# EPFL-VILAB/omnidata

Hardware: AMD Instinct MI355X
Metric: images/sec (384x384) DPT-Hybrid surface-normal inference (higher is better)
Workload: dtype bf16; 1 GPU; DPT-Hybrid-384 normal, batch 32/GPU, bf16, 1xMI355X (BASELINE.json configs[1]); batch_per_gpu=32, global_batch=32, parallelism=replicas x1 (no collective in the loop), ranks_seen=1, inflight=1

## Files before the change

include/dptx.h:

```cpp
#ifndef DPTX_H_
#define DPTX_H_

#include <stddef.h>
#include <stdint.h>

#ifdef __cplusplus
extern "C" {
#endif

typedef struct dptx_engine* dptx_handle;

enum {
  DPTX_OK = 0,
  DPTX_E_INVALID = -1,
  DPTX_E_KEY = -2,
  DPTX_E_HIP = -3,
  DPTX_E_NODEVICE = -4,
  DPTX_E_ALLOC = -5
};

enum { DPTX_DTYPE_BF16 = 0, DPTX_DTYPE_FP16 = 1, DPTX_DTYPE_BF16X3 = 2,
       DPTX_DTYPE_FP16X3 = 3, DPTX_DTYPE_MIXED = 4,
       DPTX_DTYPE_FP8 = 5 };
enum { DPTX_GROUP_RESNET = 1,
// ... 221 lines not shown
int dptx_op_cls_rows(int32_t dtype, const float* cls, const float* pos, float* X, int32_t B, int32_t S, int32_t C, void* X16,
                     float* row_stats, void* X8, float q_scale, void* stream);
int dptx_debug_set_trace(void* dev_buf);
int dptx_debug_arena_fill(dptx_handle h, int32_t byte_value);
int dptx_debug_arena_read(dptx_handle h, void* dst_host, size_t offset, size_t bytes);
int dptx_debug_arena_layout(dptx_handle h, char* dst, size_t capacity);
int dptx_debug_arena_checksums(dptx_handle h, void* out_dev, int32_t capacity, void* stream);
int dptx_debug_set_gemm_flags(int32_t flags);
int dptx_op_conv_fp8(const void* X8, const void* Wt8, const float* bias, const void* R, void* Y, void* Y8, int32_t B,
                     int32_t H, int32_t W, int32_t Cin, int32_t Cout, int32_t ksize, int32_t stride, int32_t pad_t,
                     int32_t pad_l, int32_t Ho, int32_t Wo, int32_t act, int32_t q_relu, float out_scale, void* stream);
int dptx_op_conv_groupnorm(int32_t dtype, const void* X, const void* Wt, void* Yraw, const float* gamma, const float* beta,
                           const void* R, void* Y, int32_t B, int32_t H, int32_t W, int32_t Cin, int32_t Cout,
                           int32_t ksize, int32_t stride, int32_t pad_t, int32_t pad_l, int32_t Ho, int32_t Wo,
                           int32_t relu, float eps, void* scratch_f32, void* stream);
int dptx_op_upsample2x(int32_t dtype, const void* X, void* Y, int32_t B, int32_t H, int32_t W,
                       int32_t C, void* stream);
int dptx_op_gemm_ln(int32_t dtype, const void* A, const void* W, const float* bias, void* C, int32_t M, int32_t N, int32_t K,
                    int32_t act, const float* ln_stats, const float* ln_colsum, int32_t ln_nblk, float ln_eps, void* stream);
int dptx_op_gemm_stream(int32_t dtype, const void* A, const void* W, const float* bias, void* C, float* row_stats, int32_t M,
                        int32_t N, int32_t K, void* stream);
int dptx_op_gemm_stream32(int32_t dtype, const void* A, const void* W, const float* bias, float* X, void* C16, float* row_stats,
                          int32_t M, int32_t N, int32_t K, void* stream);
int dptx_op_head_tail(int32_t dtype, const void* H0, const void* W2, const float* b2, const float* w4,
                      const float* b4, float* y, int32_t B, int32_t Hs, int32_t Ws, int32_t C,
                      int32_t relu_out, void* stream);

typedef struct dptx_unet_engine* dptx_unet_handle;
typedef struct dptx_unet_config {
  int32_t out_channels;
// ... 40 lines not shown
```

omnidata_amd/csrc/conv1x1.hip:

```cpp
#include "gemm_impl.h"

namespace dptx {

constexpr int C1_STG_PITCH = 144;
constexpr int C1_STG_WAVE = 16 * C1_STG_PITCH;
constexpr int C1_WAVES = 4;

template <int KT, int BN>
constexpr size_t conv1x1_smem_bytes() {
  return (size_t)KT * BN * 128 + (size_t)C1_WAVES * KT * 32 * 128 + (size_t)C1_WAVES * C1_STG_WAVE;
}

template <int DT, int KT, int BN>
__global__ __launch_bounds__(64 * C1_WAVES, KT <= 2 ? 2 : 1) void conv1x1_stream_kernel(const GemmParams p) {
#if defined(__HIP_DEVICE_COMPILE__)
  constexpr int NSUB = BN / 64;
  constexpr int KS = KT * 4;
  constexpr int W_BYTES = KT * BN * 128;
  constexpr int A_WAVE = KT * 32 * 128;
  extern __shared__ __attribute__((aligned(16))) char smem[];

  const int tid = threadIdx.x;
  const int lane = tid & 63;
  const int wave = __builtin_amdgcn_readfirstlane(tid >> 6);
  const int lr = lane & 31, lh = lane >> 5;

  const int npan = p.N / BN;
  const int x = (int)blockIdx.x & 7, l = (int)blockIdx.x >> 3;
// ... 35 lines not shown
    }
  };

  if (rb < rb_total) issue_a(rb);
  for (int idx = wave; idx < KT * (BN / 8); idx += C1_WAVES) {
    const int kt = idx / (BN / 8), rg = idx - kt * (BN / 8);
    const int row = rg * 8 + r0;
    const unsigned vo = (unsigned)(((long long)(n0 + row) * p.ldw + kt * 64 + (kc ^ ((row >> 1) & 7)) * 8) * 2);
    __builtin_amdgcn_raw_ptr_buffer_load_lds(rsrcW, (__attribute__((address_space(3))) void*)(sw + kt * (BN * 128) + rg * 1024), 16, vo,
                                             0, 0, 0);
  }
  float bias_c[NSUB][2];
#pragma unroll
  for (int s = 0; s < NSUB; ++s)
#pragma unroll
    for (int j = 0; j < 2; ++j) bias_c[s][j] = p.bias != nullptr ? p.bias[n0 + s * 64 + j * 32 + lr] : 0.f;
  asm volatile("s_waitcnt vmcnt(0)" ::: "memory");
  __syncthreads();

  const int swz = (lr >> 1) & 7;
  const unsigned sel = (lr & 1) ? 0x03020706u : 0x05040100u;
  const int cn = lane & 7, rr = lane >> 3;

  for (; rb < rb_total; rb += slots) {
    const int m0 = rb * 32;
    u32x4_t af[KS];
#pragma unroll
    for (int ks = 0; ks < KS; ++ks)
      af[ks] = *(const u32x4_t*)(sa + (ks >> 2) * 4096 + lr * 128 + (((2 * (ks & 3) + lh) ^ swz) << 4));
    asm volatile("s_waitcnt lgkmcnt(0)" ::: "memory");
    const bool prefetch = rb + slots < rb_total;
    if (prefetch) issue_a(rb + slots);

#pragma unroll
    for (int s = 0; s < NSUB; ++s) {
      f32x16_t acc[1][2];
#pragma unroll
      for (int j = 0; j < 2; ++j)
#pragma unroll
        for (int r = 0; r < 16; ++r) acc[0][j][r] = 0.f;
// ... 3 lines not shown
#pragma unroll
        for (int q = 0; q < 4; ++q)
#pragma unroll
          for (int j = 0; j < 2; ++j)
            bf[q][j] = *(const u32x4_t*)(sw + kt * (BN * 128) + (s * 64 + j * 32 + lr) * 128 + (((2 * q + lh) ^ swz) << 4));
        __builtin_amdgcn_sched_barrier(0);
#pragma unroll
        for (int q = 0; q < 4; ++q)
#pragma unroll
          for (int j = 0; j < 2; ++j) acc[0][j] = T16<DT>::mfma32(af[kt * 4 + q], bf[q][j], acc[0][j]);
      }
      if (s == 0) {
        __builtin_amdgcn_sched_barrier(0);
        asm volatile("s_waitcnt vmcnt(0)" ::: "memory");
      }
      if (p.gn_part != nullptr) gn_records<1, 2>(p, m0, n0 + s * 64, 0, 0, lr, lh, acc);

#pragma unroll
      for (int h = 0; h < 2; ++h) {
        asm volatile("" ::: "memory");
        __builtin_amdgcn_wave_barrier();
#pragma unroll
        for (int j = 0; j < 2; ++j)
#pragma unroll
          for (int t = 0; t < 4; ++t) {
            float v0 = acc[0][j][8 * h + 2 * t] + bias_c[s][j], v1 = acc[0][j][8 * h + 2 * t + 1] + bias_c[s][j];
            if (p.act == 1) { v0 = fmaxf(v0, 0.f); v1 = fmaxf(v1, 0.f); }
            const uint32_t own = T16<DT>::pack2(v0, v1);
            const uint32_t nb = (uint32_t)__builtin_amdgcn_update_dpp(0, (int)own, 0xB1, 0xf, 0xf, false);
            const uint32_t o = __builtin_amdgcn_perm(nb, own, sel);
            const int rl = ((2 * t) & 3) + (lr & 1) + 8 * (t >> 1) + 4 * lh;
            *(uint32_t*)(stg + rl * C1_STG_PITCH + (j * 32 + (lr & ~1)) * 2) = o;
          }
        asm volatile("" ::: "memory");
        __builtin_amdgcn_wave_barrier();
#pragma unroll
        for (int pp = 0; pp < 2; ++pp) {
          const int rl = rr + 8 * pp;
          const u32x4_t d = *(const u32x4_t*)(stg + rl * C1_STG_PITCH + cn * 16);
          const int m = m0 + 16 * h + rl;
          if (m < p.M) *(u32x4_t*)((uint16_t*)p.C + (long long)(p.c_row_off + m) * p.ldc + (n0 + s * 64 + cn * 8)) = d;
        }
      }
    }
  }
#endif
}

bool conv1x1_stream_eligible(int mode, const GemmParams& p) {
  if (mode != MODE_BF16 && mode != MODE_FP16) return false;
  if (p.ksz != 1 || p.pad_t != 0 || p.pad_l != 0 || (p.stride != 1 && p.stride != 2)) return false;
  if (p.K != p.Cin || (p.K != 64 && p.K != 128 && p.K != 256) || p.N % 64 != 0) return false;
  if (p.a_fp32 || p.c_fp32 || p.epi2 || p.a_relu || p.R1 != nullptr || p.R2 != nullptr || p.bias_per_img) return false;
  if (p.c_rpi != 0x7fffffff || p.C8 != nullptr || p.C16 != nullptr || p.out_scale != 0.f) return false;
  if (p.row_stats != nullptr || p.ln_stats != nullptr || (p.act != 0 && p.act != 1)) return false;
  if (p.ldc % 8 != 0 || p.a_pix_stride % 8 != 0 || p.a_off % 8 != 0 || p.a_img_stride % 8 != 0) return false;
  if (p.a_bytes <= 0 || p.a_bytes >= (1ll << 31) || (long long)p.N * p.ldw * 2 >= (1ll << 31) || p.M >= (1 << 23)) return false;
  return true;
}

bool conv1x1_stream_adopted(const GemmParams& p) {
  if (p.stride != 1) return false;
  if (p.K == 64) return p.N == 256 || p.N == 64;
  if (p.K == 128) return p.N == 512;
  if (p.K == 256) return p.N == 64 || p.N == 128 || (p.N == 256 && p.a_rpi >= 48 * 48);
  return false;
}

template <int DT, int KT, int BN>
static hipError_t launch_c1(const GemmParams& p, hipStream_t stream) {
  constexpr size_t smem = conv1x1_smem_bytes<KT, BN>();
  static_assert(smem <= 160 * 1024 && (KT > 2 || 2 * smem <= 160 * 1024), "two blocks per CU at K <= 128");
  const int npan = p.N / BN;
  const int rb_total = (p.M + 31) / 32;
  const int want = (rb_total + C1_WAVES - 1) / C1_WAVES;
  int cap = (KT <= 2 ? 512 : 256) / npan;
  if (cap < 8) cap = 8;
  int groups = want < cap ? want : cap;
  groups = (groups + 7) / 8 * 8;
  auto k = conv1x1_stream_kernel<DT, KT, BN>;
  set_smem_attr(k, smem);
  hipLaunchKernelGGL(k, dim3(groups * npan), dim3(64 * C1_WAVES), smem, stream, p);
  return hipGetLastError();
}

template <int DT>
static hipError_t launch_c1_dt(const GemmParams& p, hipStream_t stream) {
  if (p.K == 64) {
    if (p.N % 256 == 0) return launch_c1<DT, 1, 256>(p, stream);
    if (p.N % 128 == 0) return launch_c1<DT, 1, 128>(p, stream);
    return launch_c1<DT, 1, 64>(p, stream);
  }
  if (p.K == 128) return p.N % 128 == 0 ? launch_c1<DT, 2, 128>(p, stream) : launch_c1<DT, 2, 64>(p, stream);
  return p.N % 128 == 0 ? launch_c1<DT, 4, 128>(p, stream) : launch_c1<DT, 4, 64>(p, stream);
}

hipError_t launch_conv1x1_stream(int mode, const GemmParams& p, hipStream_t stream) {
  if (!conv1x1_stream_eligible(mode, p)) return hipErrorInvalidValue;
  return mode == MODE_BF16 ? launch_c1_dt<DT_BF16>(p, stream) : launch_c1_dt<DT_FP16>(p, stream);
}

}
```

omnidata_amd/csrc/engine.hip:

```cpp
#include <hip/hip_runtime.h>

#include <algorithm>
#include <cmath>
#include <cstdio>
#include <chrono>
#include <cstring>
#include <map>
#include <memory>
#include <string>
#include <unordered_map>
#include <vector>

#include "../../include/dptx.h"
#include "kernels.h"

using namespace dptx;

namespace {

constexpr int IMG = 384;
constexpr int S_TOK = 577;
constexpr int FEAT = 256;
const int STAGE_DEPTH[3] = {3, 4, 9};
const int STAGE_OUT[3] = {256, 512, 1024};
// ... 353 lines not shown
  double cat_ms[4] = {0, 0, 0, 0};
  int64_t cat_launches[4] = {0, 0, 0, 0};
  double cat_macs[4] = {0, 0, 0, 0};

  static constexpr int MAX_STREAMS = 4;
  int n_streams = 2;
  bool auto_streams = false, split_tuned = false, split_on = false;
  float tune_ms_single = 0.f, tune_ms_split = 0.f;
  int force_schedule = -1;
  int half_batch = 0;
  size_t half_region = 0;
  hipStream_t sub_stream[MAX_STREAMS] = {nullptr, nullptr, nullptr, nullptr};
  hipEvent_t ev_fork = nullptr, ev_join[MAX_STREAMS] = {nullptr, nullptr, nullptr, nullptr};
  int max_h = 384, max_w = 384;
  Buf pos_alt;
  Buf sraw, stem, S[3], T1, T2, PA, PB, DS, part[4], X, Hn, QKV, AO, F1, R3, R4, L3, T4, L4, clsb, lrn[4], tA, tB,
      tC, P[4], H0, H0U, H1, lnst;
  std::vector<std::pair<std::string, const Buf*>> arena_bufs;

  int fail(int code, const std::string& m) {
    err = m;
    return code;
  }
  const void* w(const std::string& key) const { return d_blob + packed_off.at(key); }
  const float* f(const std::string& key) const { return (const float*)(d_blob + packed_off.at(key)); }
  BlobHeader blob_header() const {
    BlobHeader hd;
    memset(&hd, 0, sizeof hd);
    memcpy(hd.magic, "DPTXBLOB", 8);
    hd.version = BLOB_VERSION;
    hd.dtype = cfg.dtype; hd.backbone = backbone; hd.dual_task = cfg.dual_task; hd.num_channels = cfg.num_channels;
// ... 35 lines not shown
    if (half) b.off2 = off; else { b.off = off; b.bytes = bytes; e->arena_bufs.push_back({name, &b}); }
    off += bytes;
  };
  auto idx = [](const char* name, int i) { return name + std::to_string(i); };
  take("sraw", e->sraw, B * p2 * 64, 2);
  take("stem", e->stem, B * p4 * 64, 2);
  take("S0", e->S[0], B * p4 * 256, 2);
  take("S1", e->S[1], B * p8 * 512, 2);
  take("S2", e->S[2], B * p16 * 1024, 2);
  take("T1", e->T1, B * p4 * 128, 2);
  take("T2", e->T2, B * p4 * 64, 2);
  take("PA", e->PA, B * p4 * 256, 2);
  take("PB", e->PB, B * p4 * 256, 2);
  take("DS", e->DS, B * p4 * 256, 2);
  for (int i = 0; i < 4; ++i) take(idx("part", i), e->part[i], B * (std::max(p2 / 256, p4 / 32) + 64) * 64, 4);
  take("X", e->X, B * S * DV, 4);
  take("lnst", e->lnst, B * S * 8 * 2, 4);
  take("Hn", e->Hn, B * S * DV, 2);
  take("QKV", e->QKV, B * S * 3 * DV, 2);
  take("AO", e->AO, B * S * DV, 2);
  take("F1", e->F1, B * S * (size_t)e->dm, 2);
  take("R3", e->R3, B * p16 * DV, 2);
  take("R4", e->R4, B * p16 * DV, 2);
  take("L3", e->L3, B * p16 * DV, 2);
  take("T4", e->T4, B * p16 * DV, 2);
  take("L4", e->L4, B * p32 * DV, 2);
  take("clsb", e->clsb, B * DV, 4);
  take("pos_alt", e->pos_alt, S * DV, 4);
  const size_t rn_px[4] = {p4, p8, p16, p32};
  for (int i = 0; i < 4; ++i) take(idx("lrn", i), e->lrn[i], B * rn_px[i] * FEAT, 2);
// ... 308 lines not shown
  }

  static bool gn_fusable(int HW) { return HW % 32 == 0; }
  void gn_stats(const void* X, float* part, int HW, int C) { chk(launch_gn_stats(dt, X, part, B, HW, C, e->pl, st), "gn_stats", 2); }
  void gn_apply(void* X, const std::string& nkey, float* part, int HW, int C, int relu, const void* R = nullptr,
                const std::string& rkey = "", const float* rpart = nullptr) {
    GnParams g{};
    g.nrec = gn_fusable(HW) ? HW / 32 : 0;
    g.X = X; g.Y = X; g.gamma = e->f(nkey + ".weight"); g.beta = e->f(nkey + ".bias"); g.partial = part;
    g.R = R;
    if (!rkey.empty()) { g.r_gamma = e->f(rkey + ".weight"); g.r_beta = e->f(rkey + ".bias"); g.r_partial = rpart; }
    g.B = B; g.HW = HW; g.C = C; g.relu = relu; g.eps = 1e-5f;
    chk(launch_gn_apply(dt, g, e->pl, st), nkey.c_str(), 2);
  }

  void rcu(const std::string& p, const void* x, int H, int W, void* tmp, void* out, const GemmOpt& o) {
    const int mid_lo = e->mixed() ? (int)e->layer_reads_lo(p + "conv2.weight", cur_group) : -1;
    conv(x, H, W, FEAT, p + "conv1.weight", 3, 1, 1, 1, H, W, FEAT, tmp,
         GemmOpt().bias(e->f(p + "conv1.bias")).act(1).a_relu(1).q(e->fp8_use(p + "conv2.weight") ? 1 : 0).out_lo(mid_lo));
    conv(tmp, H, W, FEAT, p + "conv2.weight", 3, 1, 1, 1, H, W, FEAT, out,
         GemmOpt().bias(e->f(p + "conv2.bias")).R1(x).R2(o.R2_).q(o.q_).out_lo(e->mixed() ? o.out_lo_ : -1));
  }

  int forward(const void* x, void* y, void* y2);
};

int Run::forward(const void* x, void* y, void* y2) {
  dptx_engine* E = e;
  E->taps.clear();
  E->event_cat.clear();
// ... 43 lines not shown
      const int stride = (b == 0) ? STAGE_STRIDE[s] : 1;
      const int Ho = H / stride, Wo = Wd / stride;
      void* out = (b == STAGE_DEPTH[s] - 1) ? (void*)A(E->S[s]) : (void*)((b & 1) ? A(E->PB) : A(E->PA));
      const bool f_in = gn_fusable(H * Wd), f_out = gn_fusable(Ho * Wo);
      if (b == 0) {
        conv(cur, H, Wd, cin, p + "downsample.conv.weight", 1, stride, 0, 0, Ho, Wo, cout, A(E->DS), GemmOpt().gn_part(f_out ? part3 : nullptr));
        if (!f_out) gn_stats(A(E->DS), part3, Ho * Wo, cout);
      }
      conv(cur, H, Wd, cin, p + "conv1.weight", 1, 1, 0, 0, H, Wd, mid, A(E->T1), GemmOpt().gn_part(f_in ? part0 : nullptr));
      if (!f_in) gn_stats(A(E->T1), part0, H * Wd, mid);
      gn_apply(A(E->T1), p + "norm1", part0, H * Wd, mid, 1);
      const int pad = (stride == 1) ? 1 : 0;
      conv(A(E->T1), H, Wd, mid, p + "conv2.weight", 3, stride, pad, pad, Ho, Wo, mid, A(E->T2), GemmOpt().gn_part(f_out ? part1 : nullptr));
      if (!f_out) gn_stats(A(E->T2), part1, Ho * Wo, mid);
      gn_apply(A(E->T2), p + "norm2", part1, Ho * Wo, mid, 1);
      conv(A(E->T2), Ho, Wo, mid, p + "conv3.weight", 1, 1, 0, 0, Ho, Wo, cout, out, GemmOpt().gn_part(f_out ? part2 : nullptr));
      if (!f_out) gn_stats(out, part2, Ho * Wo, cout);
      if (b == 0)
        gn_apply(out, p + "norm3", part2, Ho * Wo, cout, 1, A(E->DS), p + "downsample.norm", part3);
      else
        gn_apply(out, p + "norm3", part2, Ho * Wo, cout, 1, cur);
      cur = out;
      H = Ho;
      Wd = Wo;
      cin = cout;
    }
    const char* names[3] = {"s0", "s1", "s2"};
    tap(names[s], cur, H, Wd, cout);
  }
  }

  float* X = (float*)A(E->X);
  float* lnst = (float*)A(E->lnst);
  const int ln_nblk = D_VIT / 128;
  const bool s16 = E->stream16;
  group(DPTX_GROUP_EMBED);
// ... 913 lines not shown
```

omnidata_amd/csrc/gemm.hip:

```cpp
#include "gemm_impl.h"

namespace dptx {

hipError_t launch_gemm_16(int dt, const GemmParams& p, hipStream_t stream) {
  return dt == DT_BF16 ? launch_dt<DT_BF16, 1>(p, stream) : launch_gemm_fp16(p, stream);
}

void gemm_params_dense(GemmParams& p, int M, int N, int K) {
  p = GemmParams{};
  p.M = M; p.N = N; p.K = K; p.ldw = K;
  p.a_rpi = M > 0 ? M : 1; p.Wout = p.a_rpi; p.Hin = 1; p.Win = p.a_rpi; p.Cin = K; p.a_pix_stride = K;
  p.a_img_stride = 0; p.a_off = 0; p.ksz = 1; p.stride = 1; p.pad_t = 0; p.pad_l = 0;
  p.c_rpi = 0x7fffffff; p.c_img_rows = 0; p.c_row_off = 0; p.ldc = N;
  p.a_bytes = (long long)M * K * 2;
}

void gemm_params_conv(GemmParams& p, int B, int Hin, int Win, int Cin, int Cout, int ksz, int stride, int pad_t, int pad_l,
                      int Hout, int Wout, int a_elem_bytes) {
  p = GemmParams{};
  p.M = B * Hout * Wout; p.N = Cout; p.K = ksz * ksz * Cin; p.ldw = p.K;
  p.a_rpi = Hout * Wout; p.Wout = Wout; p.Hin = Hin; p.Win = Win; p.Cin = Cin; p.a_pix_stride = Cin;
  p.a_img_stride = (long long)Hin * Win * Cin; p.a_off = 0; p.ksz = ksz; p.stride = stride; p.pad_t = pad_t; p.pad_l = pad_l;
  p.c_rpi = 0x7fffffff; p.c_img_rows = 0; p.c_row_off = 0; p.ldc = Cout;
  p.a_bytes = (long long)B * Hin * Win * Cin * a_elem_bytes;
  p.k_tap_fast = (ksz == 3 && Cin >= 512) ? 1 : 0;
}

static thread_local long long* g_trace = nullptr;
void gemm_set_trace(long long* dev_buf) { g_trace = dev_buf; }
static thread_local int g_debug_flags = 0;
void gemm_set_debug_flags(int flags) { g_debug_flags = flags; }
static thread_local float g_cu_share = 1.0f;
void gemm_set_cu_share(float share) { g_cu_share = share > 0.f && share <= 1.f ? share : 1.0f; }

hipError_t launch_gemm(int mode, const GemmParams& p0, hipStream_t stream) {
  GemmParams p = p0;
  p.trace = g_trace;
  p.debug_flags = g_debug_flags;
  if (p.cu_share <= 0.f) p.cu_share = g_cu_share;
  p.a_rpi_rcp = 1.0f / (float)(p.a_rpi > 0 ? p.a_rpi : 1);
  p.wout_rcp = 1.0f / (float)(p.Wout > 0 ? p.Wout : 1);
  if (p.gn_part != nullptr && (p.gn_hw % 32 != 0 || p.N % 32 != 0 || p.gn_cpg != p.N / 32 || p.gn_cpg < 2 || p.gn_cpg > 32 ||
                               (p.gn_cpg & (p.gn_cpg - 1)) != 0 || p.bias != nullptr || p.act != 0))
    return hipErrorInvalidValue;
  if (p.row_stats != nullptr && (p.N % 128 != 0 || p.stats_nblk != 8 || p.N / 128 > 8)) return hipErrorInvalidValue;
  if (p.ln_stats != nullptr && (p.R1 != nullptr || p.R2 != nullptr || p.bias_per_img || p.ln_colsum == nullptr || (p.ln_nblk != 6 && p.ln_nblk != 8) ||
// ... 19 lines not shown
```

omnidata_amd/csrc/kernels.h:

```cpp
#pragma once
#include <hip/hip_runtime.h>
#include <stdint.h>

#include "common.h"

namespace dptx {

void ensure_dyn_smem(const void* kernel, size_t bytes);

struct GemmParams {
  const void* A;
  const void* W;
  void* C;
  const float* bias;
  const void* R1;
  const void* R2;
  int M, N, K;
  int ldw;
  int a_rpi, Wout, Hin, Win, Cin, a_pix_stride;
  long long a_img_stride, a_off;
  long long a_bytes;
  int ksz, stride, pad_t, pad_l;
  int c_rpi, c_img_rows, c_row_off, ldc;
  int r2_bcast;
// ... 13 lines not shown
  int gn_hw, gn_blocks, gn_cpg;
  void* C8;
  int q_relu;
  float out_scale, q_scale;
  const float* out_scale_v;
  void* C16;
  float* row_stats;
  int stats_nblk;
  const float* ln_stats;
  const float* ln_colsum;
  int ln_nblk;
  float ln_eps, ln_inv_dim;
  long long* trace;
  int debug_flags;
  float a_rpi_rcp, wout_rcp;
};

void gemm_params_dense(GemmParams& p, int M, int N, int K);
void gemm_params_conv(GemmParams& p, int B, int Hin, int Win, int Cin, int Cout, int ksz, int stride, int pad_t, int pad_l,
                      int Hout, int Wout, int a_elem_bytes);
hipError_t launch_gemm(int dtype, const GemmParams& p, hipStream_t stream);
void gemm_set_trace(long long* dev_buf);
void gemm_set_debug_flags(int flags);
bool conv1x1_stream_eligible(int mode, const GemmParams& p);
bool conv1x1_stream_adopted(const GemmParams& p);
hipError_t launch_conv1x1_stream(int mode, const GemmParams& p, hipStream_t stream);
void gemm_set_cu_share(float share);

hipError_t launch_attention(int mode, const void* qkv, void* out, int B, int S, int heads, Planes pl, hipStream_t stream);

hipError_t launch_layernorm(int mode, const float* x, const float* gamma, const float* beta, void* y,
                            int M, int C, float eps, Planes pl, hipStream_t stream);

struct GnParams {
  const void* X; void* Y;
  const float* gamma; const float* beta;
  float* partial;
  const void* R;
  const float* r_gamma; const float* r_beta; const float* r_partial;
  int B, HW, C, relu;
  float eps;
  int nrec;
};
int gn_chunks(int HW, int C);
hipError_t launch_gn_stats(int mode, const void* X, float* partial, int B, int HW, int C, Planes pl, hipStream_t stream);
hipError_t launch_gn_apply(int mode, const GnParams& p, Planes pl, hipStream_t stream);
hipError_t launch_gn_relu_maxpool(int mode, const void* X, void* Y, const float* gamma, const float* beta,
                                  const float* partial, int B, int H, int W, int C, float eps, Planes pl, hipStream_t stream);

hipError_t launch_stem_conv(int mode, const void* x, int io, const void* Wt, void* y, int B, int H, int W, Planes pl,
                            hipStream_t stream);

hipError_t launch_upsample2x(int mode, const void* X, void* Y, int B, int H, int W, int C, Planes pl, hipStream_t stream,
                             void* Y8 = nullptr, float q_scale = 1.0f, bool out_hi_only = false);
hipError_t launch_amax(int mode, const void* X, size_t n, int relu, unsigned* amax_bits, hipStream_t stream);

hipError_t launch_nonfinite_scan(int mode, const void* X, size_t n, unsigned* flag, hipStream_t stream);

// ... 23 lines not shown
```

omnidata_amd/csrc/norm.hip:

```cpp
#include "common.h"
#include "kernels.h"

namespace dptx {

template <int DT, int PL, int VPL>
__global__ __launch_bounds__(256) void layernorm_kernel(const float* __restrict__ x, const float* __restrict__ gamma,
                                                        const float* __restrict__ beta, uint16_t* __restrict__ y,
                                                        int M, int C, float eps, long long plane) {
  const int lane = threadIdx.x & 63;
  const int row = blockIdx.x * 4 + (threadIdx.x >> 6);
  if (row >= M) return;
  const float* xr = x + (long long)row * C;
  float4 v[VPL];
  float s = 0.f;
#pragma unroll
  for (int j = 0; j < VPL; ++j) {
    v[j] = *(const float4*)(xr + (j * 64 + lane) * 4);
    s += (v[j].x + v[j].y) + (v[j].z + v[j].w);
  }
  const float mean = wave_sum(s) / (float)C;
  float q = 0.f;
#pragma unroll
  for (int j = 0; j < VPL; ++j) {
    const float a = v[j].x - mean, b = v[j].y - mean, c = v[j].z - mean, d = v[j].w - mean;
// ... 123 lines not shown
  __syncthreads();
  if (tid < GN_G) {
    double ss = 0.0, qq = 0.0;
#pragma unroll
    for (int sl = 0; sl < 8; ++sl) { ss += sred[sl][tid][0]; qq += sred[sl][tid][1]; }
    const double n = (double)HW * (double)cpg;
    const double mean = ss / n;
    double var = qq / n - mean * mean;
    if (var < 0.0) var = 0.0;
    smr[2 * tid] = (float)mean;
    smr[2 * tid + 1] = (float)(1.0 / sqrt(var + (double)eps));
  }
  __syncthreads();
  for (int c = tid; c < C; c += blockDim.x) {
    const int g = c / cpg;
    const float a = smr[2 * g + 1] * gamma[c];
    sa[c] = a;
    sd[c] = beta[c] - smr[2 * g] * a;
  }
  __syncthreads();
}

template <int DT, int PL>
__global__ __launch_bounds__(256) void gn_apply_kernel(const GnParams p, int pix, int nrec, long long plane) {
  __shared__ float sa[1024], sd[1024], ra[1024], rd[1024], smr[64];
  const int b = blockIdx.y;
  gn_affine_to_lds(p.partial, nrec, b, p.gamma, p.beta, p.C, p.HW, p.eps, sa, sd, smr);
  const bool r_gn = (p.R != nullptr) && (p.r_gamma != nullptr);
  if (r_gn) gn_affine_to_lds(p.r_partial, nrec, b, p.r_gamma, p.r_beta, p.C, p.HW, p.eps, ra, rd, smr);
  const int cvec = p.C >> 3;
  const int pbeg = blockIdx.x * pix;
  const int pend = min(pbeg + pix, p.HW);
  const long long img = (long long)b * p.HW * p.C;
  const uint16_t* X = (const uint16_t*)p.X + img;
  const uint16_t* R = p.R ? (const uint16_t*)p.R + img : nullptr;
  uint16_t* Y = (uint16_t*)p.Y + img;
  const int total = (pend - pbeg) * cvec;
  for (int i = threadIdx.x; i < total; i += 256) {
    const int pi = i / cvec, v = i - pi * cvec;
    const long long off = (long long)(pbeg + pi) * p.C + v * 8;
    float f[8];
    load8f<DT, PL>(X + off, plane, f);
#pragma unroll
    for (int e = 0; e < 8; ++e) f[e] = f[e] * sa[v * 8 + e] + sd[v * 8 + e];
    if (R != nullptr) {
      float r[8];
      load8f<DT, PL>(R + off, plane, r);
      if (r_gn) {
#pragma unroll
        for (int e = 0; e < 8; ++e) r[e] = r[e] * ra[v * 8 + e] + rd[v * 8 + e];
      }
#pragma unroll
      for (int e = 0; e < 8; ++e) f[e] += r[e];
    }
    if (p.relu) {
#pragma unroll
      for (int e = 0; e < 8; ++e) f[e] = fmaxf(f[e], 0.f);
    }
    store8f<DT, PL>(Y + off, plane, f);
  }
}

hipError_t launch_gn_apply(int mode, const GnParams& p, Planes pl, hipStream_t stream) {
  if (p.C % 64 != 0 || p.C > 1024) return hipErrorInvalidValue;
  const int nch = gn_chunks(p.HW, p.C);
  const int nrec = p.nrec > 0 ? p.nrec : nch;
  int nb = nch;
  if (p.nrec > 0) {
    int want = 1024 / (p.B > 0 ? p.B : 1);
    want = want < 4 ? 4 : want;
    nb = nch < want ? nch : want;
  }
  const int pix = (p.HW + nb - 1) / nb;
  dim3 grid((p.HW + pix - 1) / pix, p.B);
  DPTX_DISPATCH_MODE(mode, hipLaunchKernelGGL((gn_apply_kernel<DT, PL>), grid, dim3(256), 0, stream, p, pix, nrec, pl.act));
  return hipGetLastError();
}

template <int DT, int PL>
__global__ __launch_bounds__(256) void gn_relu_maxpool_kernel(const uint16_t* __restrict__ X, uint16_t* __restrict__ Y,
                                                              const float* __restrict__ gamma, const float* __restrict__ beta,
                                                              const float* __restrict__ partial, int nchunks, int H, int W,
                                                              int C, float eps, long long plane) {
  __shared__ float sa[1024], sd[1024], smr[64];
  const int b = blockIdx.y;
  gn_affine_to_lds(partial, nchunks, b, gamma, beta, C, H * W, eps, sa, sd, smr);
  const int Ho = (H + 1) / 2, Wo = (W + 1) / 2;
  const int cvec = C >> 3;
  const int total = Ho * Wo * cvec;
  const uint16_t* Xi = X + (long long)b * H * W * C;
// ... 39 lines not shown
```

omnidata_amd/csrc/ops.hip:

```cpp
#include <hip/hip_runtime.h>

#include "../../include/dptx.h"
#include "kernels.h"

using namespace dptx;

extern "C" {

static int rc(hipError_t r) { return r == hipSuccess ? DPTX_OK : DPTX_E_HIP; }

static Planes g_op_planes{0, 0};
int dptx_op_set_planes(int64_t act_plane_elems, int64_t w_plane_elems) {
  g_op_planes.act = act_plane_elems;
  g_op_planes.w = w_plane_elems;
  return DPTX_OK;
}

int dptx_op_gemm(int32_t dtype, const void* A, const void* W, const float* bias, const void* R, void* C, int32_t M, int32_t N,
                 int32_t K, int32_t act, int32_t a_fp32, int32_t c_fp32, int32_t r_fp32, void* stream) {
  GemmParams p;
  gemm_params_dense(p, M, N, K);
  p.A = A; p.W = W; p.C = C; p.bias = bias; p.R1 = R; p.act = act; p.a_fp32 = a_fp32; p.c_fp32 = c_fp32; p.r1_fp32 = r_fp32;
  p.planes = g_op_planes;
  return rc(launch_gemm(dtype, p, (hipStream_t)stream));
// ... 111 lines not shown
                           const void* R, void* Y, int32_t B, int32_t H, int32_t W, int32_t Cin, int32_t Cout, int32_t ksize,
                           int32_t stride, int32_t pad_t, int32_t pad_l, int32_t Ho, int32_t Wo, int32_t relu, float eps,
                           void* scratch_f32, void* stream) {
  if (scratch_f32 == nullptr || (Ho * Wo) % 32 != 0) return DPTX_E_INVALID;
  GemmParams p;
  gemm_params_conv(p, B, H, W, Cin, Cout, ksize, stride, pad_t, pad_l, Ho, Wo, 2);
  p.A = X; p.W = Wt; p.C = Yraw; p.planes = g_op_planes;
  p.gn_part = (float*)scratch_f32; p.gn_hw = Ho * Wo; p.gn_blocks = Ho * Wo / 32; p.gn_cpg = Cout / 32;
  if (launch_gemm(dtype, p, (hipStream_t)stream) != hipSuccess) return DPTX_E_HIP;
  GnParams g{};
  g.X = Yraw; g.Y = Y; g.gamma = gamma; g.beta = beta; g.partial = (float*)scratch_f32; g.R = R;
  g.B = B; g.HW = Ho * Wo; g.C = Cout; g.relu = relu; g.eps = eps; g.nrec = Ho * Wo / 32;
  return rc(launch_gn_apply(dtype, g, g_op_planes, (hipStream_t)stream));
}

int dptx_op_upsample2x(int32_t dtype, const void* X, void* Y, int32_t B, int32_t H, int32_t W, int32_t C, void* stream) {
  return rc(launch_upsample2x(dtype, X, Y, B, H, W, C, g_op_planes, (hipStream_t)stream));
}

}
```

omnidata_amd/engine.py:

```python
from __future__ import annotations

import ctypes as C
import os
from typing import Dict, Optional, Tuple

import numpy as np
import torch

_HERE = os.path.dirname(os.path.abspath(__file__))
LIB_PATH = os.environ.get("DPTX_LIB") or os.path.join(_HERE, "libdptx.so")

DTYPES = {"bf16": 0, "fp16": 1, "bf16x3": 2, "fp16x3": 3, "mixed": 4, "fp8": 5}
TWO_PLANE_DTYPES = frozenset(("bf16x3", "fp16x3", "mixed", "fp8"))
GROUPS = {"resnet": 1, "embed": 2, "vit": 4, "reassemble": 8, "rn": 16, "fusion": 32, "head": 64, "all": 127}
FLAGS = {"no_ln_fold": 1, "group_policy": 2, "fp32_stream": 4, "no_range_check": 8, "fp8_all": 16, "fp8_vit": 32}


def groups_mask(names) -> int:
    if isinstance(names, int):
        return names
    if isinstance(names, str):
        names = [n for n in names.replace(",", "+").split("+") if n]
    mask = 0
    for n in names:
# ... 94 lines not shown
    ("dptx_op_conv_planes", C.c_int, [_i32, _vp, _vp, _vp, _vp, _vp] + [_i32] * 16 + [_vp]),
    ("dptx_op_stem_conv", C.c_int, [_i32, _vp, _vp, _vp, _i32, _i32, _i32, _vp]),
    ("dptx_op_attention", C.c_int, [_i32, _vp, _vp, _i32, _i32, _i32, _vp]),
    ("dptx_op_layernorm", C.c_int, [_i32, _vp, _vp, _vp, _vp, _i32, _i32, C.c_float, _vp]),
    ("dptx_op_groupnorm", C.c_int, [_i32, _vp, _vp, _vp, _vp, _vp, _i32, _i32, _i32, _i32, C.c_float, _vp, _vp]),
    ("dptx_op_gn_relu_maxpool", C.c_int, [_i32, _vp, _vp, _vp, _vp, _i32, _i32, _i32, _i32, C.c_float, _vp, _vp]),
    ("dptx_op_cls_rows", C.c_int, [_i32, _vp, _vp, _vp, _i32, _i32, _i32, _vp, _vp, _vp, C.c_float, _vp]),
    ("dptx_debug_set_trace", C.c_int, [_vp]),
    ("dptx_debug_set_gemm_flags", C.c_int, [C.c_int32]),
    ("dptx_debug_arena_fill", C.c_int, [_vp, _i32]),
    ("dptx_debug_arena_read", C.c_int, [_vp, _vp, _sz, _sz]),
    ("dptx_debug_arena_layout", C.c_int, [_vp, C.c_char_p, _sz]),
    ("dptx_debug_arena_checksums", C.c_int, [_vp, _vp, _i32, _vp]),
    ("dptx_op_conv_fp8", C.c_int, [_vp, _vp, _vp, _vp, _vp, _vp] + [_i32] * 13 + [C.c_float, _vp]),
    ("dptx_op_conv_groupnorm", C.c_int, [_i32, _vp, _vp, _vp, _vp, _vp, _vp, _vp] + [_i32] * 12 + [C.c_float, _vp, _vp]),
    ("dptx_op_upsample2x", C.c_int, [_i32, _vp, _vp, _i32, _i32, _i32, _i32, _vp]),
    ("dptx_op_gemm_ln", C.c_int, [_i32, _vp, _vp, _vp, _vp, _i32, _i32, _i32, _i32, _vp, _vp, _i32, C.c_float, _vp]),
    ("dptx_op_gemm_stream", C.c_int, [_i32, _vp, _vp, _vp, _vp, _vp, _i32, _i32, _i32, _vp]),
    ("dptx_op_gemm_stream32", C.c_int, [_i32, _vp, _vp, _vp, _vp, _vp, _vp, _i32, _i32, _i32, _vp]),
    ("dptx_op_head_tail", C.c_int, [_i32, _vp, _vp, _vp, _vp, _vp, _vp, _i32, _i32, _i32, _i32, _i32, _vp]),
    ("dptx_unet_default_config", None, [_vp]),
    ("dptx_unet_create", C.c_int, [C.POINTER(_vp), _vp]),
    ("dptx_unet_destroy", None, [_vp]),
    ("dptx_unet_last_error", C.c_char_p, [_vp]),
    ("dptx_unet_load_tensor", C.c_int, [_vp, C.c_char_p, _vp, _i64p, _i32]),
    ("dptx_unet_finalize_weights", C.c_int, [_vp]),
    ("dptx_unet_packed_bytes", _sz, [_vp]),
    ("dptx_unet_packed_entry", C.c_int, [_vp, C.c_char_p, _i64p, _i64p]),
    ("dptx_unet_export_packed_host", C.c_int, [_vp, _vp, _sz]),
    ("dptx_unet_device_bytes", _sz, [_vp]),
# ... 368 lines not shown
```

Baseline: 2823 images/s.

## Fold GroupNorm into 1x1 conv via stats pass and recompute-with-epilogue pass

For ResNet bottleneck conv3 (1x1) layers, the conv is run twice: first a stats-only pass that writes only GroupNorm partial records, then a small finalize kernel builds per-image scale/shift tables, then the conv is recomputed with an epilogue that applies the GN affine, the residual (optionally with its own GN), and ReLU before writing. This removes the write and re-read of the raw conv output and the separate gn_apply pass, at the cost of doubling the 1x1 conv arithmetic. It is limited to K=64/N=256 and K=128/N=512 shapes. The gn_apply kernel also switches to explicit fma/add rounding so its results match the fused path.

Measured after the change: 2868 images/s, median of 6. +1.6%, better.

```diff
diff --git a/include/dptx.h b/include/dptx.h
--- a/include/dptx.h
+++ b/include/dptx.h
@@ -259,6 +259,10 @@
                            const void* R, void* Y, int32_t B, int32_t H, int32_t W, int32_t Cin, int32_t Cout,
                            int32_t ksize, int32_t stride, int32_t pad_t, int32_t pad_l, int32_t Ho, int32_t Wo,
                            int32_t relu, float eps, void* scratch_f32, void* stream);
+int dptx_op_conv_groupnorm_fused(int32_t dtype, const void* X, const void* Wt, const float* gamma, const float* beta,
+                                 const void* R, const float* r_gamma, const float* r_beta, const float* r_records, void* Y,
+                                 int32_t B, int32_t H, int32_t W, int32_t Cin, int32_t Cout, int32_t relu, float eps,
+                                 void* records_f32, void* tables_f32, int32_t passes, void* stream);
 int dptx_op_upsample2x(int32_t dtype, const void* X, void* Y, int32_t B, int32_t H, int32_t W,
                        int32_t C, void* stream);
 int dptx_op_gemm_ln(int32_t dtype, const void* A, const void* W, const float* bias, void* C, int32_t M, int32_t N, int32_t K,
diff --git a/omnidata_amd/csrc/conv1x1.hip b/omnidata_amd/csrc/conv1x1.hip
--- a/omnidata_amd/csrc/conv1x1.hip
+++ b/omnidata_amd/csrc/conv1x1.hip
@@ -11,7 +11,16 @@
   return (size_t)KT * BN * 128 + (size_t)C1_WAVES * KT * 32 * 128 + (size_t)C1_WAVES * C1_STG_WAVE;
 }
 
-template <int DT, int KT, int BN>
+template <int DT>
+__device__ __forceinline__ void c1_unpack8(const u32x4_t v, float* f) {
+#pragma unroll
+  for (int i = 0; i < 4; ++i) {
+    f[2 * i] = T16<DT>::tof((uint16_t)(v[i] & 0xffffu));
+    f[2 * i + 1] = T16<DT>::tof((uint16_t)(v[i] >> 16));
+  }
+}
+
+template <int DT, int KT, int BN, int FORM>
 __global__ __launch_bounds__(64 * C1_WAVES, KT <= 2 ? 2 : 1) void conv1x1_stream_kernel(const GemmParams p) {
 #if defined(__HIP_DEVICE_COMPILE__)
   constexpr int NSUB = BN / 64;
@@ -77,7 +86,7 @@
 #pragma unroll
   for (int s = 0; s < NSUB; ++s)
 #pragma unroll
-    for (int j = 0; j < 2; ++j) bias_c[s][j] = p.bias != nullptr ? p.bias[n0 + s * 64 + j * 32 + lr] : 0.f;
+    for (int j = 0; j < 2; ++j) bias_c[s][j] = FORM == C1_PLAIN && p.bias != nullptr ? p.bias[n0 + s * 64 + j * 32 + lr] : 0.f;
   asm volatile("s_waitcnt vmcnt(0)" ::: "memory");
   __syncthreads();
 
@@ -85,8 +94,35 @@
   const unsigned sel = (lr & 1) ? 0x03020706u : 0x05040100u;
   const int cn = lane & 7, rr = lane >> 3;
 
+  const bool has_r = FORM == C1_GN && p.R1 != nullptr;
+  const bool r_gn = has_r && p.gn_tab_rgn != 0;
+
   for (; rb < rb_total; rb += slots) {
     const int m0 = rb * 32;
+    float ga[NSUB][8], gd[NSUB][8], gra[NSUB][8], grd[NSUB][8];
+    u32x4_t rq[NSUB][4];
+    auto load_epi = [&](int s) {
+      const int img = m0 / p.gn_hw;
+      const float* tab = p.gn_tab + (long long)img * 4 * p.N + n0 + s * 64 + cn * 8;
+      if (has_r) {
+#pragma unroll
+        for (int i = 0; i < 4; ++i) {
+          const int m = m0 + 16 * (i >> 1) + rr + 8 * (i & 1);
+          rq[s][i] = *(const u32x4_t*)((const uint16_t*)p.R1 + (long long)(p.c_row_off + m) * p.ldc + (n0 + s * 64 + cn * 8));
+        }
+      }
+      *(float4*)&ga[s][0] = *(const float4*)(tab);
+      *(float4*)&ga[s][4] = *(const float4*)(tab + 4);
+      *(float4*)&gd[s][0] = *(const float4*)(tab + p.N);
+      *(float4*)&gd[s][4] = *(const float4*)(tab + p.N + 4);
+      if (r_gn) {
+        *(float4*)&gra[s][0] = *(const float4*)(tab + 2 * p.N);
+        *(float4*)&gra[s][4] = *(const float4*)(tab + 2 * p.N + 4);
+        *(float4*)&grd[s][0] = *(const float4*)(tab + 3 * p.N);
+        *(float4*)&grd[s][4] = *(const float4*)(tab + 3 * p.N + 4);
+      }
+    };
+    if (FORM == C1_GN) load_epi(0);
     u32x4_t af[KS];
 #pragma unroll
     for (int ks = 0; ks < KS; ++ks)
@@ -120,7 +156,9 @@
         __builtin_amdgcn_sched_barrier(0);
         asm volatile("s_waitcnt vmcnt(0)" ::: "memory");
       }
-      if (p.gn_part != nullptr) gn_records<1, 2>(p, m0, n0 + s * 64, 0, 0, lr, lh, acc);
+      if (FORM == C1_STATS || (FORM == C1_PLAIN && p.gn_part != nullptr)) gn_records<1, 2>(p, m0, n0 + s * 64, 0, 0, lr, lh, acc);
+      if (FORM == C1_STATS) continue;
+      if (FORM == C1_GN && s + 1 < NSUB) load_epi(s + 1);
 
 #pragma unroll
       for (int h = 0; h < 2; ++h) {
@@ -131,7 +169,7 @@
 #pragma unroll
           for (int t = 0; t < 4; ++t) {
             float v0 = acc[0][j][8 * h + 2 * t] + bias_c[s][j], v1 = acc[0][j][8 * h + 2 * t + 1] + bias_c[s][j];
-            if (p.act == 1) { v0 = fmaxf(v0, 0.f); v1 = fmaxf(v1, 0.f); }
+            if (FORM != C1_GN && p.act == 1) { v0 = fmaxf(v0, 0.f); v1 = fmaxf(v1, 0.f); }
             const uint32_t own = T16<DT>::pack2(v0, v1);
             const uint32_t nb = (uint32_t)__builtin_amdgcn_update_dpp(0, (int)own, 0xB1, 0xf, 0xf, false);
             const uint32_t o = __builtin_amdgcn_perm(nb, own, sel);
@@ -143,9 +181,31 @@
 #pragma unroll
         for (int pp = 0; pp < 2; ++pp) {
           const int rl = rr + 8 * pp;
-          const u32x4_t d = *(const u32x4_t*)(stg + rl * C1_STG_PITCH + cn * 16);
+          u32x4_t d = *(const u32x4_t*)(stg + rl * C1_STG_PITCH + cn * 16);
           const int m = m0 + 16 * h + rl;
-          if (m < p.M) *(u32x4_t*)((uint16_t*)p.C + (long long)(p.c_row_off + m) * p.ldc + (n0 + s * 64 + cn * 8)) = d;
+          if (FORM == C1_GN) {
+            float f[8];
+            c1_unpack8<DT>(d, f);
+#pragma unroll
+            for (int e = 0; e < 8; ++e) f[e] = __builtin_fmaf(f[e], ga[s][e], gd[s][e]);
+            if (has_r) {
+              float r[8];
+              c1_unpack8<DT>(rq[s][2 * h + pp], r);
+              if (r_gn) {
+#pragma unroll
+                for (int e = 0; e < 8; ++e) r[e] = __builtin_fmaf(r[e], gra[s][e], grd[s][e]);
+              }
+#pragma unroll
+              for (int e = 0; e < 8; ++e) f[e] = __fadd_rn(f[e], r[e]);
+            }
+            if (p.act == 1) {
+#pragma unroll
+              for (int e = 0; e < 8; ++e) f[e] = fmaxf(f[e], 0.f);
+            }
+#pragma unroll
+            for (int e = 0; e < 4; ++e) d[e] = T16<DT>::pack2(f[2 * e], f[2 * e + 1]);
+          }
+          if (FORM == C1_GN || m < p.M) *(u32x4_t*)((uint16_t*)p.C + (long long)(p.c_row_off + m) * p.ldc + (n0 + s * 64 + cn * 8)) = d;
         }
       }
     }
@@ -173,7 +233,20 @@
   return false;
 }
 
-template <int DT, int KT, int BN>
+bool conv1x1_gn_eligible(int mode, const GemmParams& p) {
+  if (!conv1x1_stream_eligible(mode, p) || p.stride != 1 || p.bias != nullptr || p.act != 0) return false;
+  const int cpg = p.N / 32;
+  if (p.a_rpi % 32 != 0 || p.M % p.a_rpi != 0 || p.N > 1024 || (cpg & (cpg - 1)) != 0) return false;
+  return p.c_row_off == 0 && p.ldc == p.N;
+}
+
+bool conv1x1_gn_adopted(const GemmParams& p) {
+  if (p.K == 64) return p.N == 256;
+  if (p.K == 128) return p.N == 512;
+  return false;
+}
+
+template <int DT, int KT, int BN, int FORM>
 static hipError_t launch_c1(const GemmParams& p, hipStream_t stream) {
   constexpr size_t smem = conv1x1_smem_bytes<KT, BN>();
   static_assert(smem <= 160 * 1024 && (KT > 2 || 2 * smem <= 160 * 1024), "two blocks per CU at K <= 128");
@@ -184,26 +257,48 @@
   if (cap < 8) cap = 8;
   int groups = want < cap ? want : cap;
   groups = (groups + 7) / 8 * 8;
-  auto k = conv1x1_stream_kernel<DT, KT, BN>;
+  auto k = conv1x1_stream_kernel<DT, KT, BN, FORM>;
   set_smem_attr(k, smem);
   hipLaunchKernelGGL(k, dim3(groups * npan), dim3(64 * C1_WAVES), smem, stream, p);
   return hipGetLastError();
 }
 
-template <int DT>
+template <int DT, int FORM>
 static hipError_t launch_c1_dt(const GemmParams& p, hipStream_t stream) {
   if (p.K == 64) {
-    if (p.N % 256 == 0) return launch_c1<DT, 1, 256>(p, stream);
-    if (p.N % 128 == 0) return launch_c1<DT, 1, 128>(p, stream);
-    return launch_c1<DT, 1, 64>(p, stream);
-  }
-  if (p.K == 128) return p.N % 128 == 0 ? launch_c1<DT, 2, 128>(p, stream) : launch_c1<DT, 2, 64>(p, stream);
-  return p.N % 128 == 0 ? launch_c1<DT, 4, 128>(p, stream) : launch_c1<DT, 4, 64>(p, stream);
-}
-
-hipError_t launch_conv1x1_stream(int mode, const GemmParams& p, hipStream_t stream) {
-  if (!conv1x1_stream_eligible(mode, p)) return hipErrorInvalidValue;
-  return mode == MODE_BF16 ? launch_c1_dt<DT_BF16>(p, stream) : launch_c1_dt<DT_FP16>(p, stream);
-}
-
-}
+    if constexpr (FORM != C1_GN)
+      if (p.N % 256 == 0) return launch_c1<DT, 1, 256, FORM>(p, stream);
+    if (p.N % 128 == 0) return launch_c1<DT, 1, 128, FORM>(p, stream);
+    return launch_c1<DT, 1, 64, FORM>(p, stream);
+  }
+  if (p.K == 128) return p.N % 128 == 0 ? launch_c1<DT, 2, 128, FORM>(p, stream) : launch_c1<DT, 2, 64, FORM>(p, stream);
+  return p.N % 128 == 0 ? launch_c1<DT, 4, 128, FORM>(p, stream) : launch_c1<DT, 4, 64, FORM>(p, stream);
+}
+
+template <int FORM>
+static hipError_t launch_c1_form(int mode, const GemmParams& p, hipStream_t stream) {
+  return mode == MODE_BF16 ? launch_c1_dt<DT_BF16, FORM>(p, stream) : launch_c1_dt<DT_FP16, FORM>(p, stream);
+}
+
+hipError_t launch_conv1x1_stream(int mode, const GemmParams& p0, hipStream_t stream, int form) {
+  if (form == C1_PLAIN) {
+    if (!conv1x1_stream_eligible(mode, p0) || p0.gn_tab != nullptr) return hipErrorInvalidValue;
+    return launch_c1_form<C1_PLAIN>(mode, p0, stream);
+  }
+  GemmParams p = p0;
+  p.trace = nullptr;
+  p.a_rpi_rcp = 1.0f / (float)(p.a_rpi > 0 ? p.a_rpi : 1);
+  p.wout_rcp = 1.0f / (float)(p.Wout > 0 ? p.Wout : 1);
+  GemmParams q = p;
+  q.R1 = nullptr; q.act = 0; q.gn_tab = nullptr; q.gn_tab_rgn = 0; q.r1_fp32 = 0;
+  if (p.M <= 0 || p.ldw < p.K || p.ldw % 8 != 0 || !conv1x1_gn_eligible(mode, q) || p.r1_fp32) return hipErrorInvalidValue;
+  p.gn_hw = p.a_rpi; p.gn_blocks = p.a_rpi / 32; p.gn_cpg = p.N / 32;
+  if (form == C1_STATS) {
+    if (p.gn_part == nullptr || p.R1 != nullptr || p.act != 0 || p.gn_tab != nullptr) return hipErrorInvalidValue;
+    return launch_c1_form<C1_STATS>(mode, p, stream);
+  }
+  if (form != C1_GN || p.gn_tab == nullptr || p.gn_part != nullptr || p.C == nullptr || p.C == p.R1) return hipErrorInvalidValue;
+  return launch_c1_form<C1_GN>(mode, p, stream);
+}
+
+}
diff --git a/omnidata_amd/csrc/engine.hip b/omnidata_amd/csrc/engine.hip
--- a/omnidata_amd/csrc/engine.hip
+++ b/omnidata_amd/csrc/engine.hip
@@ -391,7 +391,7 @@
   hipEvent_t ev_fork = nullptr, ev_join[MAX_STREAMS] = {nullptr, nullptr, nullptr, nullptr};
   int max_h = 384, max_w = 384;
   Buf pos_alt;
-  Buf sraw, stem, S[3], T1, T2, PA, PB, DS, part[4], X, Hn, QKV, AO, F1, R3, R4, L3, T4, L4, clsb, lrn[4], tA, tB,
+  Buf sraw, stem, S[3], T1, T2, PA, PB, DS, part[4], gntab, X, Hn, QKV, AO, F1, R3, R4, L3, T4, L4, clsb, lrn[4], tA, tB,
       tC, P[4], H0, H0U, H1, lnst;
   std::vector<std::pair<std::string, const Buf*>> arena_bufs;
 
@@ -457,6 +457,7 @@
   take("PB", e->PB, B * p4 * 256, 2);
   take("DS", e->DS, B * p4 * 256, 2);
   for (int i = 0; i < 4; ++i) take(idx("part", i), e->part[i], B * (std::max(p2 / 256, p4 / 32) + 64) * 64, 4);
+  take("gntab", e->gntab, B * 4 * 1024, 4);
   take("X", e->X, B * S * DV, 4);
   take("lnst", e->lnst, B * S * 8 * 2, 4);
   take("Hn", e->Hn, B * S * DV, 2);
@@ -795,6 +796,32 @@
     chk(launch_gn_apply(dt, g, e->pl, st), nkey.c_str(), 2);
   }
 
+  bool conv_gn_folded(const void* in, int H, int W, int Cin, const std::string& wkey, int Cout, void* out, const std::string& nkey,
+                      float* part, int relu, const void* R, const std::string& rkey = "", const float* rpart = nullptr) {
+    const int flags = gemm_debug_flags();
+    if ((flags & (8 | 32)) || !gn_fusable(H * W) || out == R || (e->fp8_use(wkey) && !e->calibrating)) return false;
+    GemmParams p;
+    gemm_params_conv(p, B, H, W, Cin, Cout, 1, 1, 0, 0, H, W, 2);
+    p.A = in; p.W = e->w(wkey); p.C = out; p.planes = e->pl;
+    if (!conv1x1_gn_eligible(dt, p) || !((flags & 64) || conv1x1_gn_adopted(p))) return false;
+    float* tab = (float*)A(e->gntab);
+    const double macs = (double)p.M / B * p.N * p.K;
+    GemmParams q = p;
+    q.gn_part = part;
+    exec_macs += macs; cat_macs[0] += macs;
+    chk(launch_conv1x1_stream(dt, q, st, C1_STATS), (wkey + ".stats").c_str(), 0);
+    const bool r_gn = !rkey.empty();
+    chk(launch_gn_finalize(part, e->f(nkey + ".weight"), e->f(nkey + ".bias"), r_gn ? rpart : nullptr,
+                           r_gn ? e->f(rkey + ".weight") : nullptr, r_gn ? e->f(rkey + ".bias") : nullptr, tab, B, H * W, Cout,
+                           H * W / 32, 1e-5f, st),
+        (nkey + ".finalize").c_str(), 2);
+    q = p;
+    q.R1 = R; q.act = relu; q.gn_tab = tab; q.gn_tab_rgn = r_gn;
+    exec_macs += macs; cat_macs[0] += macs;
+    chk(launch_conv1x1_stream(dt, q, st, C1_GN), wkey.c_str(), 0);
+    return true;
+  }
+
   void rcu(const std::string& p, const void* x, int H, int W, void* tmp, void* out, const GemmOpt& o) {
     const int mid_lo = e->mixed() ? (int)e->layer_reads_lo(p + "conv2.weight", cur_group) : -1;
     conv(x, H, W, FEAT, p + "conv1.weight", 3, 1, 1, 1, H, W, FEAT, tmp,
@@ -868,12 +895,17 @@
       conv(A(E->T1), H, Wd, mid, p + "conv2.weight", 3, stride, pad, pad, Ho, Wo, mid, A(E->T2), GemmOpt().gn_part(f_out ? part1 : nullptr));
       if (!f_out) gn_stats(A(E->T2), part1, Ho * Wo, mid);
       gn_apply(A(E->T2), p + "norm2", part1, Ho * Wo, mid, 1);
-      conv(A(E->T2), Ho, Wo, mid, p + "conv3.weight", 1, 1, 0, 0, Ho, Wo, cout, out, GemmOpt().gn_part(f_out ? part2 : nullptr));
-      if (!f_out) gn_stats(out, part2, Ho * Wo, cout);
-      if (b == 0)
-        gn_apply(out, p + "norm3", part2, Ho * Wo, cout, 1, A(E->DS), p + "downsample.norm", part3);
-      else
-        gn_apply(out, p + "norm3", part2, Ho * Wo, cout, 1, cur);
+      const bool folded = b == 0 ? conv_gn_folded(A(E->T2), Ho, Wo, mid, p + "conv3.weight", cout, out, p + "norm3", part2, 1, A(E->DS),
+                                                  p + "downsample.norm", part3)
+                                 : conv_gn_folded(A(E->T2), Ho, Wo, mid, p + "conv3.weight", cout, out, p + "norm3", part2, 1, cur);
+      if (!folded) {
+        conv(A(E->T2), Ho, Wo, mid, p + "conv3.weight", 1, 1, 0, 0, Ho, Wo, cout, out, GemmOpt().gn_part(f_out ? part2 : nullptr));
+        if (!f_out) gn_stats(out, part2, Ho * Wo, cout);
+        if (b == 0)
+          gn_apply(out, p + "norm3", part2, Ho * Wo, cout, 1, A(E->DS), p + "downsample.norm", part3);
+        else
+          gn_apply(out, p + "norm3", part2, Ho * Wo, cout, 1, cur);
+      }
       cur = out;
       H = Ho;
       Wd = Wo;
diff --git a/omnidata_amd/csrc/gemm.hip b/omnidata_amd/csrc/gemm.hip
--- a/omnidata_amd/csrc/gemm.hip
+++ b/omnidata_amd/csrc/gemm.hip
@@ -30,6 +30,7 @@
 void gemm_set_trace(long long* dev_buf) { g_trace = dev_buf; }
 static thread_local int g_debug_flags = 0;
 void gemm_set_debug_flags(int flags) { g_debug_flags = flags; }
+int gemm_debug_flags() { return g_debug_flags; }
 static thread_local float g_cu_share = 1.0f;
 void gemm_set_cu_share(float share) { g_cu_share = share > 0.f && share <= 1.f ? share : 1.0f; }
 
diff --git a/omnidata_amd/csrc/kernels.h b/omnidata_amd/csrc/kernels.h
--- a/omnidata_amd/csrc/kernels.h
+++ b/omnidata_amd/csrc/kernels.h
@@ -51,6 +51,8 @@
   long long* trace;
   int debug_flags;
   float a_rpi_rcp, wout_rcp;
+  const float* gn_tab;
+  int gn_tab_rgn;
 };
 
 void gemm_params_dense(GemmParams& p, int M, int N, int K);
@@ -59,9 +61,13 @@
 hipError_t launch_gemm(int dtype, const GemmParams& p, hipStream_t stream);
 void gemm_set_trace(long long* dev_buf);
 void gemm_set_debug_flags(int flags);
+int gemm_debug_flags();
 bool conv1x1_stream_eligible(int mode, const GemmParams& p);
 bool conv1x1_stream_adopted(const GemmParams& p);
-hipError_t launch_conv1x1_stream(int mode, const GemmParams& p, hipStream_t stream);
+enum { C1_PLAIN = 0, C1_STATS = 1, C1_GN = 2 };
+bool conv1x1_gn_eligible(int mode, const GemmParams& p);
+bool conv1x1_gn_adopted(const GemmParams& p);
+hipError_t launch_conv1x1_stream(int mode, const GemmParams& p, hipStream_t stream, int form = C1_PLAIN);
 void gemm_set_cu_share(float share);
 
 hipError_t launch_attention(int mode, const void* qkv, void* out, int B, int S, int heads, Planes pl, hipStream_t stream);
@@ -79,6 +85,9 @@
   float eps;
   int nrec;
 };
+hipError_t launch_gn_finalize(const float* partial, const float* gamma, const float* beta, const float* r_partial,
+                              const float* r_gamma, const float* r_beta, float* tab, int B, int HW, int C, int nrec, float eps,
+                              hipStream_t stream);
 int gn_chunks(int HW, int C);
 hipError_t launch_gn_stats(int mode, const void* X, float* partial, int B, int HW, int C, Planes pl, hipStream_t stream);
 hipError_t launch_gn_apply(int mode, const GnParams& p, Planes pl, hipStream_t stream);
diff --git a/omnidata_amd/csrc/norm.hip b/omnidata_amd/csrc/norm.hip
--- a/omnidata_amd/csrc/norm.hip
+++ b/omnidata_amd/csrc/norm.hip
@@ -161,9 +161,9 @@
   __syncthreads();
   for (int c = tid; c < C; c += blockDim.x) {
     const int g = c / cpg;
-    const float a = smr[2 * g + 1] * gamma[c];
+    const float a = __fmul_rn(smr[2 * g + 1], gamma[c]);
     sa[c] = a;
-    sd[c] = beta[c] - smr[2 * g] * a;
+    sd[c] = __builtin_fmaf(-a, smr[2 * g], beta[c]);
   }
   __syncthreads();
 }
@@ -189,16 +189,16 @@
     float f[8];
     load8f<DT, PL>(X + off, plane, f);
 #pragma unroll
-    for (int e = 0; e < 8; ++e) f[e] = f[e] * sa[v * 8 + e] + sd[v * 8 + e];
+    for (int e = 0; e < 8; ++e) f[e] = __builtin_fmaf(f[e], sa[v * 8 + e], sd[v * 8 + e]);
     if (R != nullptr) {
       float r[8];
       load8f<DT, PL>(R + off, plane, r);
       if (r_gn) {
 #pragma unroll
-        for (int e = 0; e < 8; ++e) r[e] = r[e] * ra[v * 8 + e] + rd[v * 8 + e];
+        for (int e = 0; e < 8; ++e) r[e] = __builtin_fmaf(r[e], ra[v * 8 + e], rd[v * 8 + e]);
       }
 #pragma unroll
-      for (int e = 0; e < 8; ++e) f[e] += r[e];
+      for (int e = 0; e < 8; ++e) f[e] = __fadd_rn(f[e], r[e]);
     }
     if (p.relu) {
 #pragma unroll
@@ -221,6 +221,27 @@
   const int pix = (p.HW + nb - 1) / nb;
   dim3 grid((p.HW + pix - 1) / pix, p.B);
   DPTX_DISPATCH_MODE(mode, hipLaunchKernelGGL((gn_apply_kernel<DT, PL>), grid, dim3(256), 0, stream, p, pix, nrec, pl.act));
+  return hipGetLastError();
+}
+
+__global__ __launch_bounds__(256) void gn_finalize_kernel(const float* __restrict__ partial, const float* __restrict__ gamma,
+                                                          const float* __restrict__ beta, const float* __restrict__ r_partial,
+                                                          const float* __restrict__ r_gamma, const float* __restrict__ r_beta,
+                                                          float* __restrict__ tab, int nrec, int C, int HW, float eps) {
+  __shared__ float smr[64];
+  const int b = blockIdx.x, t = blockIdx.y;
+  float* const ta = tab + ((long long)b * 4 + 2 * t) * C;
+  gn_affine_to_lds(t ? r_partial : partial, nrec, b, t ? r_gamma : gamma, t ? r_beta : beta, C, HW, eps, ta, ta + C, smr);
+}
+
+hipError_t launch_gn_finalize(const float* partial, const float* gamma, const float* beta, const float* r_partial,
+                              const float* r_gamma, const float* r_beta, float* tab, int B, int HW, int C, int nrec, float eps,
+                              hipStream_t stream) {
+  if (C % 64 != 0 || C > 1024 || B <= 0 || nrec <= 0 || partial == nullptr || gamma == nullptr || beta == nullptr || tab == nullptr)
+    return hipErrorInvalidValue;
+  if (r_partial != nullptr && (r_gamma == nullptr || r_beta == nullptr)) return hipErrorInvalidValue;
+  hipLaunchKernelGGL(gn_finalize_kernel, dim3(B, r_partial != nullptr ? 2 : 1), dim3(256), 0, stream, partial, gamma, beta,
+                     r_partial, r_gamma, r_beta, tab, nrec, C, HW, eps);
   return hipGetLastError();
 }
 
diff --git a/omnidata_amd/csrc/ops.hip b/omnidata_amd/csrc/ops.hip
--- a/omnidata_amd/csrc/ops.hip
+++ b/omnidata_amd/csrc/ops.hip
@@ -149,6 +149,36 @@
   return rc(launch_gn_apply(dtype, g, g_op_planes, (hipStream_t)stream));
 }
 
+int dptx_op_conv_groupnorm_fused(int32_t dtype, const void* X, const void* Wt, const float* gamma, const float* beta, const void* R,
+                                 const float* r_gamma, const float* r_beta, const float* r_records, void* Y, int32_t B, int32_t H,
+                                 int32_t W, int32_t Cin, int32_t Cout, int32_t relu, float eps, void* records_f32, void* tables_f32,
+                                 int32_t passes, void* stream) {
+  if (records_f32 == nullptr || tables_f32 == nullptr || (passes & ~7) != 0 || passes == 0 || H <= 0 || W <= 0) return DPTX_E_INVALID;
+  if ((r_gamma != nullptr) != (r_beta != nullptr) || (r_gamma != nullptr) != (r_records != nullptr)) return DPTX_E_INVALID;
+  if (r_gamma != nullptr && R == nullptr) return DPTX_E_INVALID;
+  GemmParams p;
+  gemm_params_conv(p, B, H, W, Cin, Cout, 1, 1, 0, 0, H, W, 2);
+  p.A = X; p.W = Wt; p.C = Y; p.planes = g_op_planes;
+  if (!conv1x1_gn_eligible(dtype, p)) return DPTX_E_INVALID;
+  hipStream_t st = (hipStream_t)stream;
+  if (passes & 1) {
+    GemmParams q = p;
+    q.gn_part = (float*)records_f32;
+    if (launch_conv1x1_stream(dtype, q, st, C1_STATS) != hipSuccess) return DPTX_E_HIP;
+  }
+  if (passes & 2) {
+    if (launch_gn_finalize((const float*)records_f32, gamma, beta, r_records, r_gamma, r_beta, (float*)tables_f32, B, H * W, Cout,
+                           H * W / 32, eps, st) != hipSuccess)
+      return DPTX_E_HIP;
+  }
+  if (passes & 4) {
+    GemmParams q = p;
+    q.R1 = R; q.act = relu ? 1 : 0; q.gn_tab = (const float*)tables_f32; q.gn_tab_rgn = r_gamma != nullptr;
+    if (launch_conv1x1_stream(dtype, q, st, C1_GN) != hipSuccess) return DPTX_E_HIP;
+  }
+  return DPTX_OK;
+}
+
 int dptx_op_upsample2x(int32_t dtype, const void* X, void* Y, int32_t B, int32_t H, int32_t W, int32_t C, void* stream) {
   return rc(launch_upsample2x(dtype, X, Y, B, H, W, C, g_op_planes, (hipStream_t)stream));
 }
diff --git a/omnidata_amd/engine.py b/omnidata_amd/engine.py
--- a/omnidata_amd/engine.py
+++ b/omnidata_amd/engine.py
@@ -132,6 +132,7 @@
     ("dptx_debug_arena_checksums", C.c_int, [_vp, _vp, _i32, _vp]),
     ("dptx_op_conv_fp8", C.c_int, [_vp, _vp, _vp, _vp, _vp, _vp] + [_i32] * 13 + [C.c_float, _vp]),
     ("dptx_op_conv_groupnorm", C.c_int, [_i32, _vp, _vp, _vp, _vp, _vp, _vp, _vp] + [_i32] * 12 + [C.c_float, _vp, _vp]),
+    ("dptx_op_conv_groupnorm_fused", C.c_int, [_i32] + [_vp] * 9 + [_i32] * 6 + [C.c_float, _vp, _vp, _i32, _vp]),
     ("dptx_op_upsample2x", C.c_int, [_i32, _vp, _vp, _i32, _i32, _i32, _i32, _vp]),
     ("dptx_op_gemm_ln", C.c_int, [_i32, _vp, _vp, _vp, _vp, _i32, _i32, _i32, _i32, _vp, _vp, _i32, C.c_float, _vp]),
     ("dptx_op_gemm_stream", C.c_int, [_i32, _vp, _vp, _vp, _vp, _vp, _i32, _i32, _i32, _vp]),
```
